# bioinf/Sibelia

Hardware: AMD Instinct MI355X
Metric: k-mers/sec in BlockFinder graph-build+simplify, 8xE.coli k=25 (higher is better)
Workload: dtype u64; 1 GPU; 8 synthetic E. coli-like strains x 4.6 Mbp (gen_strains seed 1, 1% SNP, indels, inversions), k=25 D=150 maxIterations=4, one full stage; strand_kmers_per_gpu=73598388, parallelism=1 GPU, exchange_bytes_rank0=0, bulges=334284, bif_ids=1120044, instances=7089276, rounds=106, replays=0, device_bytes=22762263122

## Files before the change

sibelia_amd/csrc/bulge_txn.h:

```cpp
#pragma once
#include <hip/hip_runtime.h>
#include <stdint.h>

#define BT_NONE 0xFFFFFFFFu
#define BT_SEP '$'
#define BT_DEAD_CHAR 0
#define BT_POS_MASK 0x1FFFFFFFu
#define BT_MAX_BREAKS 16u
#define BT_LDS_MARKS 48u
#define BT_BLOCK_SHIFT 0
#define BT_INSERT_ALIGN 1u
#define BT_RSHIFT 0u
#define BT_LAZY_MIN 64u
#define BT_MSCAN_MIN 6u
__host__ __device__ __forceinline__ uint32_t bt_insert_span(uint32_t m) { return (m + BT_INSERT_ALIGN - 1u) & ~(BT_INSERT_ALIGN - 1u); }

enum { CTR_STRIDE = 32,
       CTR_NE = 0 * CTR_STRIDE, CTR_NN = 1 * CTR_STRIDE, CTR_ERR = 2 * CTR_STRIDE, CTR_BULGES = 3 * CTR_STRIDE, CTR_VIOL = 4 * CTR_STRIDE,
       CTR_NWIN = 5 * CTR_STRIDE, CTR_LO = 6 * CTR_STRIDE, CTR_COMMITTED = 7 * CTR_STRIDE, CTR_BIG = 8 * CTR_STRIDE, CTR_PUSHED = 9 * CTR_STRIDE,
       CTR_TXN = 10 * CTR_STRIDE, CTR_DETAIL = 11 * CTR_STRIDE, CTR_COUNT = 12 * CTR_STRIDE };
enum { CTR_VDETAIL = CTR_DETAIL + 0, CTR_VDETAIL_N = 5,
       CTR_DENSE_ITER = CTR_DETAIL + 0,
       CTR_PARKED = CTR_DETAIL + 8,
       CTR_PLIST = CTR_DETAIL + 10,
// ... 351 lines not shown
	uint32_t mks;
	bool mk_overflow;
	uint32_t *wst; char *wck;
	uint32_t *wbk, *wnb;
	uint32_t *wdel;
	unsigned long long *dirty_big;
	bool lite;
	bool lazy;
	bool use_stale;
	unsigned long long stale[4];
	uint32_t epoch, *wep;
	uint32_t req[2], nreq;
	bool jscan, jready;
	uint32_t nold;
	bool mscan, mready;
	bool wfill; uint32_t fill_i;
	bool pscan, pready, pjknown; uint32_t pj;
	uint32_t ret0;
	uint32_t mscan_min;
	uint32_t mq_i, mq_di, mq_j, mq_dj, mres[2];
	uint64_t *visit; uint32_t nvisit, visit_cap;
	uint32_t *occ; uint32_t occ_cap;
	uint32_t *lb, *lf;
	AnyBulgesOut ab;
	ABuild abb;
	uint32_t gi, idI, idJ, ret;
	bool inI, need_fill;
	uint32_t c_src, c_dS, c_tgt, c_dT;
	uint32_t *act;
};
// ... 687 lines not shown
```

sibelia_amd/csrc/commit.hip:

```cpp
#include <cstring>
#include <algorithm>
#include <vector>
#include <hip/hip_runtime.h>
__device__ unsigned long long g_phase_cycles[32];
#if defined(__HIP_DEVICE_COMPILE__)
#define BT_PROF_T0(t) do { if ((t).prof) (t).prof_t = __builtin_readcyclecounter(); } while (0)
#define BT_PROF_ADD(t, i) do { if ((t).prof) { unsigned long long n_ = __builtin_readcyclecounter(); atomicAdd(&g_phase_cycles[i], n_ - (t).prof_t); (t).prof_t = n_; } } while (0)
#endif
#include "simplify_walks.h"

__device__ __forceinline__ void wave_stamp_id_write(const GraphView &g, unsigned stampv, unsigned tid, unsigned id, unsigned b)
{
	unsigned r = g.nblk + b;
	unsigned ow = g.own[b], wm = g.wmax[r], rm = g.rmax[r];
	bool bad = (stampv != BT_NONE && ow != stampv) || wm > tid || rm > tid;
	atomicMax(&g.wmax[r], tid);
	if (bad) {
		atomicMin(&g.ctr[CTR_VIOL], id);
		if (atomicCAS(&g.ctr[CTR_VDETAIL], 0u, 3u) == 0u) { g.ctr[CTR_VDETAIL + 1] = r; g.ctr[CTR_VDETAIL + 2] = (wm > rm ? wm : rm) - 1; g.ctr[CTR_VDETAIL + 3] = id; g.ctr[CTR_VDETAIL + 4] = (wm > tid ? 1u : 0u) | (rm > tid ? 2u : 0u) | (ow != stampv ? 4u : 0u); }
	}
}
__device__ __forceinline__ void wave_erase(const GraphView &g, Txn &t, unsigned strand, unsigned e, unsigned stampv, unsigned b, unsigned nd)
{
	if (b == BT_NONE) return;
// ... 1027 lines not shown
	WSYNC();
	PC_ADD(18);
	return sh.mode == 3;
	}
}


#define PARK_OFF_LAYOUT (PARK_IMG - 16u)
#define PARK_OFF_W ((unsigned)((sizeof(Txn) + 15u) & ~15u))
#define PARK_OFF_AB (PARK_OFF_W + (unsigned)((sizeof(BulgeWork) + 15u) & ~15u))
#define PARK_OFF_FAST (PARK_OFF_AB + (unsigned)((sizeof(ABShared) + 15u) & ~15u))
static_assert(sizeof(Txn) % 4 == 0 && sizeof(BulgeWork) % 4 == 0 && sizeof(ABShared) % 4 == 0, "park_move copies words");
static_assert(PARK_OFF_FAST + COMMIT_FAST_BYTES <= PARK_OFF_LAYOUT, "the LDS image of a transaction must fit PARK_IMG");
__device__ __forceinline__ unsigned lds_addr(const void *p) { return (unsigned)(uintptr_t)(const __attribute__((address_space(3))) void *)p; }
__device__ __forceinline__ void park_move(unsigned *dst, const unsigned *src, unsigned words, unsigned lane) { for (unsigned i = lane; i < words; i += 64) dst[i] = src[i]; }
__device__ __forceinline__ void park_store(const GraphView &g, Txn &t, BulgeWork &w, ABShared &absh, uint8_t *fast, unsigned fast_bytes, uint8_t *image, unsigned id, unsigned slice)
{
	const unsigned lane = threadIdx.x;
	WSYNC();
	park_move(reinterpret_cast<unsigned *>(image), reinterpret_cast<const unsigned *>(&t), sizeof(Txn) / 4, lane);
	park_move(reinterpret_cast<unsigned *>(image + PARK_OFF_W), reinterpret_cast<const unsigned *>(&w), sizeof(BulgeWork) / 4, lane);
	park_move(reinterpret_cast<unsigned *>(image + PARK_OFF_AB), reinterpret_cast<const unsigned *>(&absh), sizeof(ABShared) / 4, lane);
	park_move(reinterpret_cast<unsigned *>(image + PARK_OFF_FAST), reinterpret_cast<const unsigned *>(fast), fast_bytes / 4, lane);
	if (lane == 0) {
		unsigned *lay = reinterpret_cast<unsigned *>(image + PARK_OFF_LAYOUT);
		lay[0] = lds_addr(&t); lay[1] = lds_addr(&w); lay[2] = lds_addr(&absh); lay[3] = lds_addr(fast);
		g.park_of[id] = (slice + 1u) | (bt_round_tag(g) << 20); g.slice_busy[slice] = 1; g.need[id] = 2; atomicAdd(&g.ctr[CTR_PARKED], 1u);
#ifdef SBL_DBG_IDRET
		if (id < (1u << 20)) atomicCAS(&g_dbg_park[id], 0u, ((SS_ROUND_MAX - (g.round_bits >> 20)) << 8) | (w.ret & 255u));
#endif
	}
}
__device__ __forceinline__ bool park_load(const GraphView &g, Txn &t, BulgeWork &w, ABShared &absh, uint8_t *fast, unsigned fast_bytes, const uint8_t *image, unsigned id, unsigned wi, int prof)
{
	const unsigned lane = threadIdx.x;
	{
		const unsigned *lay = reinterpret_cast<const unsigned *>(image + PARK_OFF_LAYOUT);
		const bool same = lay[0] == lds_addr(&t) && lay[1] == lds_addr(&w) && lay[2] == lds_addr(&absh) && lay[3] == lds_addr(fast);
		if (!same) { if (lane == 0) atomicOr(&g.ctr[CTR_ERR], BT_ERR_LAYOUT); return false; }
	}
	park_move(reinterpret_cast<unsigned *>(&t), reinterpret_cast<const unsigned *>(image), sizeof(Txn) / 4, lane);
	park_move(reinterpret_cast<unsigned *>(&w), reinterpret_cast<const unsigned *>(image + PARK_OFF_W), sizeof(BulgeWork) / 4, lane);
	park_move(reinterpret_cast<unsigned *>(&absh), reinterpret_cast<const unsigned *>(image + PARK_OFF_AB), sizeof(ABShared) / 4, lane);
	park_move(reinterpret_cast<unsigned *>(fast), reinterpret_cast<const unsigned *>(image + PARK_OFF_FAST), fast_bytes / 4, lane);
	WSYNC();
	if (lane == 0) { t.g = g; t.stamp = g.round_bits | wi; t.prof = prof != 0; w.ret0 = w.ret - 1; atomicSub(&g.ctr[CTR_PARKED], 1u); }
	WSYNC();
	return true;
}
template <bool RESUME = false>
__device__ __forceinline__ void commit_body(const GraphView &g, Txn &t, BulgeWork &w, int &flag, ABShared &absh, uint8_t *fast, unsigned fast_bytes,
                                            unsigned wi, unsigned id, unsigned stampv, int solo, bool prepass, uint8_t *mine, unsigned arena_bytes, int prof,
                                            const unsigned *sepl = nullptr ,
                                            unsigned park_slice = BT_NONE )
{
	const unsigned lane = threadIdx.x, tid = id + 1;
	PH_T0();
	const bool can_park = park_slice != BT_NONE && g.park_cap != 0 && arena_bytes >= 4u * PARK_IMG;
	if (can_park) arena_bytes -= PARK_IMG;
	if (lane == 0) { g.need[id] = 0; g.touch[id] = 1; flag = 1; }
	if (RESUME) {
		if (!park_load(g, t, w, absh, fast, fast_bytes, mine + arena_bytes, id, wi, prof)) return;
		if (lane == 0) flag = 1;
		WSYNC();
	} else {
	if (prepass) {
		if (lane == 0) { t.init(g, id, wi, 1, mine, arena_bytes); t.ext_stamps = true; t.chain = stampv == BT_NONE; }
		WSYNC();
		wave_setup(g, t, w, true, lane, flag);
		if (flag) {
			wave_scan_all(g, w, lane, stampv, tid, 1, id);
			WSYNC();
		}
		int verdict = flag ? wave_verdict(g, w, *reinterpret_cast<VerdictTable *>(fast), lane) : 0;
		if (lane == 0) {
			bool has = verdict > 0;
			if (verdict < 0) { bt_end_chars(t, w); has = bt_any_bulges(t, w, true); }
			if (t.err & BT_ERR_SCRATCH) { atomicOr(&g.ctr[CTR_ERR], BT_ERR_SCRATCH); has = false; }
			flag = has ? 1 : 0;
		}
	}
	WSYNC();
	if (!flag) { if (lane == 0) { atomicAdd(&g.ctr[CTR_COMMITTED], 1u); atomicAdd(&g.ctr[CTR_TXN], 1u); } return; }
	if (lane == 0) { t.init(g, id, wi, 2, mine, arena_bytes); t.chain = stampv == BT_NONE; t.defer_push = true; t.ext_stamps = true; t.fscr = fast; t.fscr_cap = fast_bytes; w.ret = 0;
	                 t.tc_cap = 1024; t.tc_list = (uint32_t *)t.alloc(t.tc_cap * 4); if (!t.tc_list) t.tc_cap = 0; t.err = 0; t.defer_cleanup = true; t.prof = prof != 0; }
	WSYNC();
	PH_ADD(7);
	{
		const unsigned h0 = g.head[0][t.id], h1 = g.head[1][t.id];
		if (lane == 0) flag = bt_setup(t, w, false, false) && !t.err ? 1 : 0;
		WSYNC();
		PH_ADD(19);
		if (flag) {
			const unsigned m = wave_list_positions(g, h0, h1, w, lane);
			if (m != w.n && lane == 0) {
				if (t.g.any_parked && m < w.n) { w.n = m; if (m < 2) flag = 0; }
				else { t.err |= BT_ERR_SCRATCH; flag = 0; }
			}
			WSYNC();
		}
	}
	}
	PH_ADD(0);
	if (flag) {
		if (!RESUME) {
		wave_scan_all(g, w, lane, stampv, tid, 2, id);
		WSYNC();
		if (w.mk_overflow) {
			WSYNC();
			if (lane == 0) bt_marks_to_arena(t, w);
			WSYNC();
			if (!t.err) for (unsigned i = 0; i < w.n; i++) wave_scan_instance(g, w, i, lane, stampv, tid, 2, id);
			WSYNC();
		}
		PH_ADD(1);
		int any = wave_any_bulges(g, t, w, absh, lane, false, AB_COUNT_SLOTS, nullptr, prof);
		if (lane == 0) { flag = bt_rb_begin(t, w, any) && !t.err ? 1 : 0; w.lazy = solo && w.wep != nullptr; w.jscan = w.lazy || w.n > 24u; w.mscan = w.n > 24u;
			                 w.use_stale = !w.lazy && w.n <= 256u && w.wdel != nullptr; w.wfill = true; w.pscan = false; }
		WSYNC();
		PH_ADD(2);
		}
		bool decided = RESUME;
		while (flag) {
			if (!RESUME || !decided) {
			if (lane == 0) { const int r = bt_scratch_in_lds(w) ? bt_rb_run<true>(t, w) : bt_rb_run<false>(t, w); flag = t.err ? 0 : r; }
			WSYNC();
			PH_ADD(3);
			if (!flag) break;
			if (flag == 3) { wave_next_j(g, w, lane); PH_ADD(24); continue; }
			if (flag == 4) { wave_mults(g, t, w, lane); PH_ADD(25); continue; }
			if (flag == 5) { wave_fill_visit(t, w, g.D, lane); PH_ADD(26); if (t.err) break; continue; }
			if (flag == 2) {
				const unsigned nr = w.nreq;
				for (unsigned x = 0; x < nr; x++) wave_scan_instance(g, w, w.req[x], lane, stampv, tid, 2, id);
				WSYNC();
				if (lane == 0) for (unsigned x = 0; x < nr; x++) { if (w.lazy) w.wep[w.req[x]] = w.epoch; else w.stale[w.req[x] >> 6] &= ~(1ull << (w.req[x] & 63u)); }
				WSYNC();
				if (!w.lazy && w.mk_overflow) {
					if (lane == 0) bt_marks_to_arena(t, w);
					WSYNC();
					if (t.err) break;
					for (unsigned i = 0; i < w.n; i++) wave_scan_instance(g, w, i, lane, stampv, tid, 2, id);
					if (lane == 0) w.stale[0] = w.stale[1] = w.stale[2] = w.stale[3] = 0;
					WSYNC();
				}
				PH_ADD(8);
				continue;
			}
			}
			decided = false;
			if (can_park && !t.g.park_hold && !w.lazy && w.ret - w.ret0 > g.park_cap) {
				park_store(g, t, w, absh, fast, fast_bytes, mine + arena_bytes, id, park_slice);
				return;
			}
#ifdef SBL_DBG_IDRET
			if (lane == 0) {
				const unsigned o = atomicAdd(&g_dbg_nlog, 1u);
				if (o < (1u << 20)) { unsigned *r = g_dbg_log + (size_t)o * 8u; r[0] = id; r[1] = SS_ROUND_MAX - (g.round_bits >> 20); r[2] = w.ret; r[3] = (g.nslot[w.start[w.c_src] >> 1] << 1) | (w.start[w.c_src] & 1u); r[4] = (g.nslot[w.start[w.c_tgt] >> 1] << 1) | (w.start[w.c_tgt] & 1u); r[5] = w.c_dS; r[6] = w.c_dT; r[7] = RESUME ? 1u : 0u; }
			}
#endif
			if (w.lazy) {
				wave_collapse_any(g, t, w, lane, stampv, prof);
				PH_ADD(5);
				if (t.err) break;
				wave_publish_collapse(g, id, t.push_e, t.push_d, t.push_len, lane, sepl);
				if (lane == 0) w.epoch++;
				WSYNC();
				PH_ADD(6);
				continue;
			}
			unsigned long long dirty[4] = {0, 0, 0, 0};
			const bool big = w.n > 256, selective = !big || w.dirty_big != nullptr;
			if (selective) {
// ... 85 lines not shown
			unsigned long long dur = __builtin_readcyclecounter() - ph_start;
			unsigned bin = 0;
			while (bin < 15 && (dur >> (13 + bin))) bin++;
			atomicAdd(&g_txn_hist[w.ret < 3 ? w.ret : 3][bin], 1ull);
			if (atomicMax(&g_txn_max[0], dur) < dur) g_txn_max[1] = ((unsigned long long)w.n << 32) | w.ret;
			{
				const unsigned long long now = wall_clock64(), sl = (g.tslot >> 2) & 4095u;
				atomicMin(&g_round_span[3 * sl], ph_wall); atomicMax(&g_round_span[3 * sl + 1], now);
				atomicMax(&g_round_span[3 * sl + 2], ((now - ph_wall) << 32) | (ph_wall & 0xFFFFFFFFull));
				if (w.ret <= 1) atomicMax(&g_round_few[2 * sl], now - ph_wall);
				if (w.ret <= 2) atomicMax(&g_round_few[2 * sl + 1], now - ph_wall);
			}
			atomicMax(&g_round_max[(g.tslot >> 2) & 4095u], (dur << 24) | ((unsigned long long)(w.n < 255u ? w.n : 255u) << 16) | ((unsigned long long)(w.nold < 255u ? w.nold : 255u) << 8) | (w.ret < 255u ? w.ret : 255u));
		}
		atomicAdd(&g.ctr[CTR_COMMITTED], 1u); atomicAdd(&g.ctr[CTR_TXN], 1u);
		if (RESUME) { __threadfence(); g.slice_busy[park_slice] = 0; g.park_of[id] = 0x80000000u | (bt_round_tag(g) << 20); }
		if (t.err) {
			if (!t.wrote && t.err == BT_ERR_SCRATCH) { ss_mark_big(g, id); return; }
			atomicOr(&g.ctr[CTR_ERR], t.err);
		}
		atomicAdd(&g.ctr[CTR_BULGES], w.ret);
#ifdef SBL_DBG_IDRET
		if (id < (1u << 20)) { atomicAdd(&g_dbg_ret[id], w.ret); atomicCAS(&g_dbg_fin[id], 0u, ((SS_ROUND_MAX - (g.round_bits >> 20)) << 8) | (RESUME ? 128u : 0u) | (w.ret & 127u)); }
#endif
	}
}

template <bool RESUME_KERNEL>
__device__ __forceinline__ void commit_kernel(const GraphView &g, unsigned nwin, uint8_t *arena, unsigned arena_bytes, int solo, const unsigned *claims, const uint8_t *live, int prof_every)
{
	const int prof = prof_every && blockIdx.x % (unsigned)prof_every == 0u;
	__shared__ Txn t;
	__shared__ BulgeWork w;
	__shared__ int flag;
	__shared__ ABShared absh;
	__shared__ __attribute__((aligned(16))) uint8_t fast[COMMIT_FAST_BYTES];
	unsigned wi = blockIdx.x;
	const unsigned lane = threadIdx.x;
	if (!RESUME_KERNEL) round_stamp(g, 2);
	if (RESUME_KERNEL) {
		if (wi >= __builtin_amdgcn_readfirstlane((int)g.ctr[CTR_PLIST])) return;
		wi = (unsigned)__builtin_amdgcn_readfirstlane((int)g.park_list[wi]);
	}
	if (wi >= nwin) return;
	if (!solo && !live[wi]) return;
	const unsigned id = g.win[wi], stampv = g.round_bits | wi;
	if (!solo) {
		const unsigned *cb = claims + (size_t)wi * (CLAIM_CAP + 1);
		unsigned n = cb[0];
		bool owner = true;
		if (n <= CLAIM_CAP) {
			for (unsigned i = lane; i < n; i += 64) {
				unsigned b = cb[1 + i];
				if (b & 0x80000000u) { if (bt_order_blocked(g, b & 0x7FFFFFFFu)) owner = false; }
				else if (g.own[b] != stampv) owner = false;
			}
			owner = !__any(!owner);
		} else {
			if (lane == 0) owner = ss_owns_footprint(g, wi);
			owner = __shfl((int)owner, 0) != 0;
		}
		if (!owner) return;
	}
	__shared__ unsigned s_sep[64];
	const unsigned *sepl = g.sep && g.nsep <= 64 ? s_sep : nullptr;
	if (sepl) s_sep[lane] = lane < g.nsep ? g.sep[lane] : BT_NONE;
	if (RESUME_KERNEL) {
		const unsigned pk = (unsigned)__builtin_amdgcn_readfirstlane((int)g.park_of[id]);
		if (!pk || (pk >> 31) || ((pk >> 20) & 0x7FFu) == bt_round_tag(g)) return;
		const unsigned slice = (pk & 0xFFFFFu) - 1u;
		commit_body<true>(g, t, w, flag, absh, fast, (unsigned)sizeof fast, wi, id, stampv, 0, false, arena + (size_t)slice * arena_bytes, arena_bytes, prof, sepl, slice);
	} else {
		if (!solo && g.park_cap) {
			const unsigned pk = (unsigned)__builtin_amdgcn_readfirstlane((int)g.park_of[id]);
			if (pk && (!(pk >> 31) || ((pk >> 20) & 0x7FFu) == bt_round_tag(g))) return;
		}
		const bool shadow = !solo && g.park_cap && __builtin_amdgcn_readfirstlane((int)g.slice_busy[g.shadow_base + 64u + wi]) != 0;
		commit_body<false>(g, t, w, flag, absh, fast, (unsigned)sizeof fast, wi, id, stampv, solo, solo != 0, arena + (size_t)(shadow ? g.shadow_base + wi : wi) * arena_bytes, arena_bytes, prof, sepl,
		                   !solo && g.park_cap && !shadow ? wi : (unsigned)BT_NONE);
	}
}
__global__ void __launch_bounds__(64) __attribute__((amdgpu_waves_per_eu(4, 4))) k_commit(GraphView g, unsigned nwin, uint8_t *arena, unsigned arena_bytes, int solo, const unsigned *claims, const uint8_t *live, int prof_every)
{
	commit_kernel<false>(g, nwin, arena, arena_bytes, solo, claims, live, prof_every);
}

__global__ void __launch_bounds__(64) __attribute__((amdgpu_waves_per_eu(4, 4))) k_resume(GraphView g, unsigned nwin, uint8_t *arena, unsigned arena_bytes, const unsigned *claims, const uint8_t *live, int prof_every)
{
	commit_kernel<true>(g, nwin, arena, arena_bytes, 0, claims, live, prof_every);
}

__global__ void __launch_bounds__(256) k_park_sweep(unsigned *__restrict__ park_of, unsigned n)
{
	const unsigned i = blockIdx.x * blockDim.x + threadIdx.x;
	if (i < n && (park_of[i] >> 31)) park_of[i] = 0u;
}

__global__ void __launch_bounds__(64) k_chain(GraphView g, uint8_t *arena, unsigned arena_bytes, unsigned nwin, int prof)
{
	__shared__ Txn t;
	__shared__ BulgeWork w;
	__shared__ int flag;
	__shared__ ABShared absh;
	__shared__ __attribute__((aligned(16))) uint8_t fast[12288];
// ... 186 lines not shown
```

sibelia_amd/csrc/simplify.hip:

```cpp
#include <cstring>
#include <algorithm>
#include <array>
#include <chrono>

#include "sbl_ctx.h"
#include "sbl_prim.h"
#include "sbl_comm.h"
#include "kmer_kernels.h"
#include "simplify_driver.h"
#include "simplify_kernels.h"

static inline unsigned nblocks(size_t n, unsigned per) { return (unsigned)((n + per - 1) / per); }

struct SimplifyHandles {
	hipStream_t park_stream = nullptr; hipEvent_t park_ev[2] = {nullptr, nullptr};
	unsigned *h_ctr = nullptr;
	unsigned *d_hctr = nullptr;
	unsigned post_seq = 0;
	hipEvent_t ev[8] = {};
	std::vector<hipEvent_t> snap_ev;
	unsigned char *h_init = nullptr;
	~SimplifyHandles()
	{
		if (park_stream) (void)hipStreamDestroy(park_stream);
		for (auto &e : park_ev) if (e) (void)hipEventDestroy(e);
		if (h_ctr) (void)hipHostFree(h_ctr);
		if (h_init) (void)hipHostFree(h_init);
		for (auto &e : ev) if (e) (void)hipEventDestroy(e);
		for (auto &e : snap_ev) (void)hipEventDestroy(e);
	}
};
struct SimplifyState : SimplifyHandles {
	DevBuf ch, op, nx, pv, nodeof[2];
	DevBuf nslot, nnext, nidst, nclr, ndead, head[2], lsize[2];
	DevBuf ctr, need, big, touch, ck_touch, own, lock, rmax, wmax, win;
	DevBuf arena, snap_arena, big_arena, claims, live, robuf, bidx, instbuf, snap_list, snap_live, park_of, slice_busy, park_list;
	DevBuf ck_ch, ck_op, ck_nx, ck_pv, ck_bif[2], ck_nodeof[2], ck_nslot, ck_nnext, ck_ndead, ck_head[2], ck_lsize[2];
	DevBuf keys, skeys, selem, sorttmp, scantmp, perm, permin;
	DevBuf nmark, maux[2], iota, sel, tstamp;
	DevBuf lin, elin, lmpos[2], lmid[2], cnt1k, off1k;
// ... 304 lines not shown
			HIP_TRY(hipGetLastError());
		}
		HIP_TRY(hipEventRecord(st->snap_ev[2 * snap_used + 1], c->stream));
		snap_used++;
	}
	void snapshots_collect()
	{
		for (unsigned i = 0; i < snap_used; i++) {
			float ms = 0;
			HIP_TRY(hipEventSynchronize(st->snap_ev[2 * i + 1]));
			HIP_TRY(hipEventElapsedTime(&ms, st->snap_ev[2 * i], st->snap_ev[2 * i + 1]));
			snapshot_ms += ms;
		}
		snap_used = 0;
	}
	void reset_round_state(bool stamps_too)
	{
		if (stamps_too && g.park_cap) {
			HIP_TRY(hipMemsetAsync(st->park_of.p, 0, ((size_t)nid_ + 1) * 4, c->stream));
			HIP_TRY(hipMemsetAsync(st->slice_busy.p, 0, park_slices, c->stream));
			parked_known = 0; g.park_hold = 0;
		}
		HIP_TRY(hipMemsetAsync(st->own.p, 0xFF, ((size_t)nid_ + 1) * 4, c->stream));
		if (stamps_too) {
			HIP_TRY(hipMemsetAsync(st->rmax.p, 0, nres * 4, c->stream));
			HIP_TRY(hipMemsetAsync(st->wmax.p, 0, nres * 4, c->stream));
			if (g.bidx) k_idx_clear_stamps<<<(idx_nblk + 255) / 256, 256, 0, c->stream>>>(st->bidx.as<unsigned long long>(), idx_nblk);
		}
	}
	void clear_counters()
	{
		k_clear_counters<<<1, 256, 0, c->stream>>>(st->ctr.as<unsigned>());
// ... 50 lines not shown
		if (hipDeviceGetAttribute(&khz, hipDeviceAttributeWallClockRate, c->device) != hipSuccess || khz <= 0) khz = 100000;
		const double ms_per_tick = 1.0 / (double)khz;
		for (uint32_t r = 0; r < ts_round; r++) {
			const unsigned long long tp = h[4 * r], tr = h[4 * r + 1], tc = h[4 * r + 2];
			const bool probed = ts_kind[r] & 1, reserved = ts_kind[r] & 2;
			if (probed) { const unsigned long long next = reserved ? tr : tc; if (next > tp && tp) probe_ms += (double)(next - tp) * ms_per_tick; }
			if (reserved && tc > tr && tr) reserve_ms += (double)(tc - tr) * ms_per_tick;
			const unsigned long long te = h[4 * r + 3];
			if ((ts_kind[r] & 4) && te > tc && tc) commit_ms += (double)(te - tc) * ms_per_tick;
		}
	}
	void probe(uint32_t nwin, uint32_t round)
	{
		g.round_bits = (SS_ROUND_MAX - round) << 20;
		g.any_parked = parked_known != 0;
		begin_round();
		solo_round = false;
		if (g.tslot < TS_CAP * 4) ts_kind.back() |= 1;
		if (split_ro()) {
			uint32_t w0 = 0, w1 = nwin;
			share(nwin, &w0, &w1);
			const uint32_t R = c->comm->n;
			const uint32_t stride = (4u + (nwin + R - 1) / R + 1u + 3u) & ~3u;
			st->robuf.ensure((size_t)R * stride + 64);
			if (w1 > w0 && g.idx_probe) k_probe_idx<<<w1 - w0, 64, pidx_lds(), c->stream>>>(g, nwin, st->live.as<uint8_t>(), w0, pidx_vbits, pidx_inst, pidx_marks, nullptr, 0u, 0);
			if (w1 > w0) k_probe<<<w1 - w0, 64 * PROBE_WAVES, 0, c->stream>>>(g, nwin, st->arena.as<uint8_t>(), arena_bytes, st->live.as<uint8_t>(), w0, 0);
			k_pack_probe<<<std::max<uint32_t>(1u, (w1 - w0 + 255) / 256), 256, 0, c->stream>>>(st->ctr.as<unsigned>(), st->live.as<uint8_t>(), w0, w1, c->comm->rank, stride, st->robuf.as<uint8_t>());
			HIP_TRY(hipGetLastError());
			allgather_slots(st->robuf.as<char>(), R, stride);
			k_apply_probe<<<(nwin + 255) / 256, 256, 0, c->stream>>>(g, nwin, st->live.as<uint8_t>(), w0, w1, st->robuf.as<uint8_t>(), stride, R);
// ... 12 lines not shown
		if (g.tslot < TS_CAP * 4) ts_kind.back() |= 2;
		const unsigned seen_bits = rsv_waves <= 2 ? 10u : 11u, list_cap = rsv_waves <= 2 ? 256u : 1024u;
		const bool handed = g.idx_probe && !split_ro() && !solo_round;
		k_reserve<<<nwin, 64 * rsv_waves, ((1u << seen_bits) + rsv_waves * list_cap) * 4, c->stream>>>(g, nwin, st->claims.as<unsigned>(), st->live.as<uint8_t>(), seen_bits, list_cap,
		                                                                                               handed ? st->instbuf.as<unsigned>() : nullptr, istride(),
		                                                                                               g.park_cap ? st->arena.as<uint8_t>() : nullptr, arena_bytes);
		HIP_TRY(hipGetLastError());
	}
	void commit(uint32_t nwin, uint32_t round, bool solo)
	{
		g.round_bits = (SS_ROUND_MAX - round) << 20;
		const bool sampled = ((round + ev_phase) & 3u) == 0;
		if (g.tslot < TS_CAP * 4) ts_kind.back() |= 4;
		if (sampled) HIP_TRY(hipEventRecord(ev[2], c->stream));
		if (solo) {
			st->big_arena.ensure(big_arena_bytes);
			k_commit<<<1, 64, 0, c->stream>>>(g, 1, st->big_arena.as<uint8_t>(), big_arena_bytes, 1, nullptr, nullptr, prof);
		} else
		{
			const bool resume = g.park_cap && parked_known != 0;
			if (g.park_cap && (round & 1023u) == 0u) k_park_sweep<<<nblocks((size_t)nid_ + 1, 256), 256, 0, c->stream>>>(st->park_of.as<unsigned>(), nid_ + 1);
			if (resume) {
				HIP_TRY(hipEventRecord(st->park_ev[0], c->stream));
				HIP_TRY(hipStreamWaitEvent(st->park_stream, st->park_ev[0], 0));
				k_resume<<<std::min<uint32_t>(parked_known, nwin), 64, 0, st->park_stream>>>(g, nwin, st->arena.as<uint8_t>(), arena_bytes, st->claims.as<unsigned>(), st->live.as<uint8_t>(), prof);
				HIP_TRY(hipEventRecord(st->park_ev[1], st->park_stream));
			}
			k_commit<<<nwin, 64, 0, c->stream>>>(g, nwin, st->arena.as<uint8_t>(), arena_bytes, 0, st->claims.as<unsigned>(), st->live.as<uint8_t>(), prof);
			if (resume) HIP_TRY(hipStreamWaitEvent(c->stream, st->park_ev[1], 0));
		}
		if (sampled) HIP_TRY(hipEventRecord(ev[3], c->stream));
		timed_commit = sampled;
		HIP_TRY(hipGetLastError());
	}
	size_t park_slices = 0;
	uint32_t parked_known = 0;
	bool chain(uint32_t nwin, uint32_t round)
	{
		if (may_try_dense && ++chain_rounds >= 32u) {
			const double el = std::chrono::duration<double>(std::chrono::steady_clock::now() - t_stage).count();
			const double within = (double)last_lo / (double)(nid_ ? nid_ : 1u);
			const double progress = iter_count <= 1u ? 0.8 * within : 0.8 + 0.2 * ((double)(iter_count - 2u) + within) / (double)(max_iter_ > 1u ? max_iter_ - 1u : 1u);
			if (el > 1.0 && progress < 0.4) throw TryDense{};
		}
		if (g.park_cap && parked_known) { g.park_hold = 1; return false; }
		g.round_bits = (SS_ROUND_MAX - round) << 20;
		st->big_arena.ensure(big_arena_bytes);
		if (g.tslot < TS_CAP * 4) ts_kind.back() |= 4;
		k_chain<<<1, 64, 0, c->stream>>>(g, st->big_arena.as<uint8_t>(), big_arena_bytes, nwin, prof);
		timed_commit = false;
		HIP_TRY(hipGetLastError());
		return true;
	}
	SimplifyCounters counters()
	{
		read_ctr();
		if (sel_pending) sel_ready = true;
		float ms = 0;
		if (timed_commit) {
			hipError_t e = hipEventElapsedTime(&ms, ev[2], ev[3]);
			if (e == hipErrorNotReady) { HIP_TRY(hipEventSynchronize(ev[3])); e = hipEventElapsedTime(&ms, ev[2], ev[3]); }
			HIP_TRY(e);
			commit_event_ms += ms; commit_event_launches++; timed_commit = false;
		}
		SimplifyCounters r;
		memcpy(r.v, st->h_ctr, sizeof r.v);
		parked_known = r.v[CTR_PARKED];
		return r;
	}
	bool grow(uint32_t err)
	{
		if (err & ~(uint32_t)(BT_ERR_ELEM_CAP | BT_ERR_NODE_CAP)) return false;
		if (optimistic) {
			if (err & BT_ERR_ELEM_CAP) c->hint_elem_slack = std::max<size_t>(c->hint_elem_slack, 2 * ((size_t)cap_e - ne0_));
// ... 207 lines not shown
		be.ev_phase = c->stage_seq++;
		be.prof = sw.phases;
		if (be.prof) sbl_commit_prof_reset();
		if (dense) be.use_index = false;
		be.idx_nblk = be.use_index ? (uint32_t)((E + 63) / 64) : 0u;
		if (be.idx_nblk) st->bidx.ensure((size_t)be.idx_nblk * BT_IDX_WORDS * 8);
		be.bind();
		be.g.k = k; be.g.D = D;
	}

	void setup_park()
	{
		be.g.park_cap = park_cap; be.g.park_of = nullptr; be.g.slice_busy = nullptr; be.g.shadow_base = 0; be.park_slices = 0;
		be.g.park_hold = 0; be.g.any_parked = 0; be.g.park_list = nullptr;
		if (!park_cap) return;
		if (!st->park_stream) { HIP_TRY(hipStreamCreateWithFlags(&st->park_stream, hipStreamNonBlocking)); for (auto &e : st->park_ev) HIP_TRY(hipEventCreateWithFlags(&e, hipEventDisableTiming)); }
		st->park_of.ensure(((size_t)be.nid_ + 1) * 4);
		be.park_slices = (size_t)window_max + 64;
		be.g.park_of = st->park_of.as<unsigned>(); be.g.slice_busy = st->slice_busy.as<uint8_t>(); be.g.shadow_base = window_max;
		be.g.park_list = st->park_list.as<unsigned>();
	}

	bool run_dense(SimplifyReport &rep, sbl_progress_fn progress, void *user)
	{
		be.g.lazy_min = 1;
		st->big_arena.ensure(be.big_arena_bytes);
		unsigned *d_out = st->ctr.as<unsigned>() + CTR_DENSE_ITER;
		HIP_TRY(hipEventRecord(be.ev[2], s));
		k_dense_stage<<<1, 64, 0, s>>>(be.g, st->big_arena.as<uint8_t>(), be.big_arena_bytes, max_iter, d_out);
		HIP_TRY(hipEventRecord(be.ev[3], s));
		HIP_TRY(hipGetLastError());
// ... 179 lines not shown
```

sibelia_amd/csrc/simplify_kernels.h:

```cpp
#pragma once
#include "sbl_ctx.h"
#include "simplify_steps.h"

#define CLAIM_CAP 4096u
#define PROBE_WAVES 1u
#define PROBE_UNSERVED 3u
#define SEL_THREADS 256
#define RSV_WAVES_MAX 4u
struct MarkStream { const unsigned *elem[2], *id[2], *aux[2]; unsigned n[2]; };

void sbl_commit_prof_reset();
void sbl_commit_prof_report(unsigned ts_round);
void sbl_rounds_stats_report();

__global__ void __launch_bounds__(256) k_init_links(unsigned *__restrict__ nx, unsigned *__restrict__ pv, unsigned *__restrict__ nodeof0,
                                                    unsigned *__restrict__ nodeof1, uint8_t *__restrict__ ch, size_t E, size_t cap);
__global__ void __launch_bounds__(256) k_instance_keys(const unsigned *__restrict__ elem, const unsigned *__restrict__ id, unsigned n, unsigned strand,
                                                       const unsigned *__restrict__ sepidx, unsigned nchr, unsigned E, unsigned ordbits,
                                                       unsigned long long *__restrict__ keys, unsigned *__restrict__ midx);
__global__ void __launch_bounds__(256) k_build_lists(const unsigned long long *__restrict__ skeys, const unsigned *__restrict__ smidx, const unsigned *__restrict__ melem, unsigned n,
                                                     unsigned node_base, unsigned strand, unsigned ordbits, unsigned *__restrict__ nslot, unsigned *__restrict__ nnext, unsigned *__restrict__ nidst,
                                                     uint8_t *__restrict__ ndead, unsigned *__restrict__ head, unsigned *__restrict__ lsize,
                                                     unsigned *__restrict__ nodeof, unsigned *__restrict__ nmark);
__global__ void __launch_bounds__(256) k_id_position_keys(const unsigned *__restrict__ head0, const unsigned *__restrict__ head1, const unsigned *__restrict__ nslot,
// ... 14 lines not shown
__global__ void __launch_bounds__(64) k_snapshot(GraphView g, uint8_t *arena, unsigned arena_bytes, int incremental, const unsigned *__restrict__ perm, unsigned plo, unsigned phi);
__global__ void __launch_bounds__(64) k_probe_idx(GraphView g, unsigned nwin, uint8_t *live, unsigned w0, unsigned vbits, unsigned max_inst, unsigned walk_marks,
                                                  unsigned *__restrict__ instbuf, unsigned istride, int snapshot);
__global__ void __launch_bounds__(64 * PROBE_WAVES) k_probe(GraphView g, unsigned nwin, uint8_t *arena, unsigned arena_bytes, uint8_t *live, unsigned w0, int snapshot);
__global__ void __launch_bounds__(256) k_pack_need(const unsigned *__restrict__ perm, const uint8_t *__restrict__ need, unsigned lo, unsigned hi, uint8_t *__restrict__ buf);
__global__ void __launch_bounds__(256) k_unpack_need(const unsigned *__restrict__ perm, const uint8_t *__restrict__ buf, unsigned n, unsigned mylo, unsigned myhi, uint8_t *__restrict__ need);
__global__ void __launch_bounds__(256) k_apply_probe(GraphView g, unsigned nwin, uint8_t *__restrict__ live, unsigned w0, unsigned w1, const uint8_t *__restrict__ robuf, unsigned stride, unsigned nranks);
__global__ void __launch_bounds__(SEL_THREADS) k_select_count(GraphView g, unsigned *__restrict__ sel, unsigned lo, unsigned limit, unsigned chunk0, unsigned chunk,
                                                              const uint8_t *__restrict__ live, unsigned probed);
__global__ void __launch_bounds__(SEL_THREADS) k_select_write(GraphView g, unsigned *__restrict__ sel, unsigned *__restrict__ win, unsigned lo, unsigned limit, unsigned W,
                                                              unsigned chunk0, unsigned chunk, unsigned nchunks, volatile unsigned *post, unsigned post_seq);
__global__ void __launch_bounds__(256) k_pack_probe(const unsigned *__restrict__ ctr, const uint8_t *__restrict__ live, unsigned w0, unsigned w1, unsigned rank, unsigned stride, uint8_t *__restrict__ robuf);
__global__ void __launch_bounds__(64 * RSV_WAVES_MAX) k_reserve(GraphView g, unsigned nwin, unsigned *claims, const uint8_t *live, unsigned seen_bits, unsigned list_cap,
                                                                 const unsigned *__restrict__ instbuf, unsigned istride, const uint8_t *arena, unsigned arena_bytes);
__global__ void __launch_bounds__(64) __attribute__((amdgpu_waves_per_eu(4, 4))) k_commit(GraphView g, unsigned nwin, uint8_t *arena, unsigned arena_bytes, int solo, const unsigned *claims, const uint8_t *live, int prof);
__global__ void __launch_bounds__(64) __attribute__((amdgpu_waves_per_eu(4, 4))) k_resume(GraphView g, unsigned nwin, uint8_t *arena, unsigned arena_bytes, const unsigned *claims, const uint8_t *live, int prof);
__global__ void __launch_bounds__(256) k_park_sweep(unsigned *__restrict__ park_of, unsigned n);
__global__ void __launch_bounds__(64) k_chain(GraphView g, uint8_t *arena, unsigned arena_bytes, unsigned nwin, int prof);
__global__ void __launch_bounds__(64) k_dense_stage(GraphView g, uint8_t *arena, unsigned arena_bytes, unsigned max_iter, unsigned *out);
__global__ void __launch_bounds__(256) k_count_touched(const uint8_t *__restrict__ touch, unsigned nid, unsigned *__restrict__ out);
__global__ void __launch_bounds__(256) k_touched_list(const uint8_t *__restrict__ touch, unsigned nid, unsigned *__restrict__ list, unsigned *__restrict__ count);
__global__ void __launch_bounds__(256) k_seg_flags(const uint8_t *__restrict__ ch, const unsigned *__restrict__ nx, unsigned ne, unsigned *__restrict__ flag);
__global__ void __launch_bounds__(256) k_seg_tails(const uint8_t *__restrict__ ch, const unsigned *__restrict__ nx, unsigned ne,
                                                   const unsigned *__restrict__ flag, const unsigned *__restrict__ segidx ,
                                                   unsigned *__restrict__ seg_head, unsigned *__restrict__ seg_len, unsigned *__restrict__ seg_succ_elem);
__global__ void __launch_bounds__(256) k_seg_finish(unsigned nseg, const unsigned *__restrict__ seg_head, unsigned *__restrict__ seg_len,
                                                    const unsigned *__restrict__ seg_succ_elem, const unsigned *__restrict__ flag,
                                                    const unsigned *__restrict__ segidx, unsigned *__restrict__ succ, unsigned long long *__restrict__ dist);
__global__ void __launch_bounds__(256) k_seg_jump(unsigned nseg, const unsigned *__restrict__ succ_in, const unsigned long long *__restrict__ dist_in,
                                                  unsigned *__restrict__ succ_out, unsigned long long *__restrict__ dist_out);
__global__ void __launch_bounds__(256) k_scatter_linear(const uint8_t *__restrict__ ch, const unsigned *__restrict__ op, unsigned ne,
// ... 19 lines not shown
```

Before: 1.310 billion strand-k-mers/s.

## Merge resume kernel into commit kernel and drop separate park stream

The separate k_resume kernel, which ran on its own stream with event handoffs, is folded into k_commit. The first blocks of the combined grid resume parked transactions and the rest run fresh windows. Resume/park state moves from a template parameter into runtime fields on BulgeWork, and the GraphView is read through the kernarg pointer. Park sweep is moved into the round-reset and round-start paths. The aim is to remove the extra stream, event record/wait and a launch per round, at the cost of runtime branching and register pressure in a single unified kernel.

Result: faster. 1.373 billion strand-k-mers/s, median of 6 (+4.8%).

```diff
diff --git a/sibelia_amd/csrc/bulge_txn.h b/sibelia_amd/csrc/bulge_txn.h
--- a/sibelia_amd/csrc/bulge_txn.h
+++ b/sibelia_amd/csrc/bulge_txn.h
@@ -389,6 +389,8 @@
 	bool jscan, jready;
 	uint32_t nold;
 	bool mscan, mready;
+	uint8_t resumed;
+	bool can_park;
 	bool wfill; uint32_t fill_i;
 	bool pscan, pready, pjknown; uint32_t pj;
 	uint32_t ret0;
diff --git a/sibelia_amd/csrc/commit.hip b/sibelia_amd/csrc/commit.hip
--- a/sibelia_amd/csrc/commit.hip
+++ b/sibelia_amd/csrc/commit.hip
@@ -1065,10 +1065,11 @@
 static_assert(PARK_OFF_FAST + COMMIT_FAST_BYTES <= PARK_OFF_LAYOUT, "the LDS image of a transaction must fit PARK_IMG");
 __device__ __forceinline__ unsigned lds_addr(const void *p) { return (unsigned)(uintptr_t)(const __attribute__((address_space(3))) void *)p; }
 __device__ __forceinline__ void park_move(unsigned *dst, const unsigned *src, unsigned words, unsigned lane) { for (unsigned i = lane; i < words; i += 64) dst[i] = src[i]; }
-__device__ __forceinline__ void park_store(const GraphView &g, Txn &t, BulgeWork &w, ABShared &absh, uint8_t *fast, unsigned fast_bytes, uint8_t *image, unsigned id, unsigned slice)
+__device__ __forceinline__ void park_store(const GraphView &g, Txn &t, BulgeWork &w, ABShared &absh, uint8_t *fast, unsigned fast_bytes, unsigned id)
 {
 	const unsigned lane = threadIdx.x;
 	WSYNC();
+	uint8_t *image = t.scr + t.scr_cap;
 	park_move(reinterpret_cast<unsigned *>(image), reinterpret_cast<const unsigned *>(&t), sizeof(Txn) / 4, lane);
 	park_move(reinterpret_cast<unsigned *>(image + PARK_OFF_W), reinterpret_cast<const unsigned *>(&w), sizeof(BulgeWork) / 4, lane);
 	park_move(reinterpret_cast<unsigned *>(image + PARK_OFF_AB), reinterpret_cast<const unsigned *>(&absh), sizeof(ABShared) / 4, lane);
@@ -1076,6 +1077,7 @@
 	if (lane == 0) {
 		unsigned *lay = reinterpret_cast<unsigned *>(image + PARK_OFF_LAYOUT);
 		lay[0] = lds_addr(&t); lay[1] = lds_addr(&w); lay[2] = lds_addr(&absh); lay[3] = lds_addr(fast);
+		const unsigned slice = w.resumed ? (g.park_of[id] & 0xFFFFFu) - 1u : t.stamp & 0xFFFFFu;
 		g.park_of[id] = (slice + 1u) | (bt_round_tag(g) << 20); g.slice_busy[slice] = 1; g.need[id] = 2; atomicAdd(&g.ctr[CTR_PARKED], 1u);
 #ifdef SBL_DBG_IDRET
 		if (id < (1u << 20)) atomicCAS(&g_dbg_park[id], 0u, ((SS_ROUND_MAX - (g.round_bits >> 20)) << 8) | (w.ret & 255u));
@@ -1095,22 +1097,22 @@
 	park_move(reinterpret_cast<unsigned *>(&absh), reinterpret_cast<const unsigned *>(image + PARK_OFF_AB), sizeof(ABShared) / 4, lane);
 	park_move(reinterpret_cast<unsigned *>(fast), reinterpret_cast<const unsigned *>(image + PARK_OFF_FAST), fast_bytes / 4, lane);
 	WSYNC();
-	if (lane == 0) { t.g = g; t.stamp = g.round_bits | wi; t.prof = prof != 0; w.ret0 = w.ret - 1; atomicSub(&g.ctr[CTR_PARKED], 1u); }
+	if (lane == 0) { t.g = g; t.stamp = g.round_bits | wi; t.prof = prof != 0; w.ret0 = w.ret - 1; w.resumed = 3; atomicSub(&g.ctr[CTR_PARKED], 1u); }
 	WSYNC();
 	return true;
 }
-template <bool RESUME = false>
 __device__ __forceinline__ void commit_body(const GraphView &g, Txn &t, BulgeWork &w, int &flag, ABShared &absh, uint8_t *fast, unsigned fast_bytes,
                                             unsigned wi, unsigned id, unsigned stampv, int solo, bool prepass, uint8_t *mine, unsigned arena_bytes, int prof,
                                             const unsigned *sepl = nullptr ,
-                                            unsigned park_slice = BT_NONE )
+                                            bool own_slice = false ,
+                                            bool resume = false )
 {
 	const unsigned lane = threadIdx.x, tid = id + 1;
 	PH_T0();
-	const bool can_park = park_slice != BT_NONE && g.park_cap != 0 && arena_bytes >= 4u * PARK_IMG;
+	const bool can_park = (own_slice || resume) && g.park_cap != 0 && arena_bytes >= 4u * PARK_IMG;
 	if (can_park) arena_bytes -= PARK_IMG;
 	if (lane == 0) { g.need[id] = 0; g.touch[id] = 1; flag = 1; }
-	if (RESUME) {
+	if (resume) {
 		if (!park_load(g, t, w, absh, fast, fast_bytes, mine + arena_bytes, id, wi, prof)) return;
 		if (lane == 0) flag = 1;
 		WSYNC();
@@ -1133,7 +1135,7 @@
 	}
 	WSYNC();
 	if (!flag) { if (lane == 0) { atomicAdd(&g.ctr[CTR_COMMITTED], 1u); atomicAdd(&g.ctr[CTR_TXN], 1u); } return; }
-	if (lane == 0) { t.init(g, id, wi, 2, mine, arena_bytes); t.chain = stampv == BT_NONE; t.defer_push = true; t.ext_stamps = true; t.fscr = fast; t.fscr_cap = fast_bytes; w.ret = 0;
+	if (lane == 0) { t.init(g, id, wi, 2, mine, arena_bytes); t.chain = stampv == BT_NONE; t.defer_push = true; t.ext_stamps = true; t.fscr = fast; t.fscr_cap = fast_bytes; w.ret = 0; w.resumed = 0; w.can_park = can_park;
 	                 t.tc_cap = 1024; t.tc_list = (uint32_t *)t.alloc(t.tc_cap * 4); if (!t.tc_list) t.tc_cap = 0; t.err = 0; t.defer_cleanup = true; t.prof = prof != 0; }
 	WSYNC();
 	PH_ADD(7);
@@ -1154,7 +1156,7 @@
 	}
 	PH_ADD(0);
 	if (flag) {
-		if (!RESUME) {
+		if (!w.resumed) {
 		wave_scan_all(g, w, lane, stampv, tid, 2, id);
 		WSYNC();
 		if (w.mk_overflow) {
@@ -1171,10 +1173,11 @@
 		WSYNC();
 		PH_ADD(2);
 		}
-		bool decided = RESUME;
 		while (flag) {
-			if (!RESUME || !decided) {
-			if (lane == 0) { const int r = bt_scratch_in_lds(w) ? bt_rb_run<true>(t, w) : bt_rb_run<false>(t, w); flag = t.err ? 0 : r; }
+			if (lane == 0) {
+				if (w.resumed & 2u) { w.resumed = 1; flag = 1; }
+				else { const int r = bt_scratch_in_lds(w) ? bt_rb_run<true>(t, w) : bt_rb_run<false>(t, w); flag = t.err ? 0 : r; }
+			}
 			WSYNC();
 			PH_ADD(3);
 			if (!flag) break;
@@ -1198,16 +1201,14 @@
 				PH_ADD(8);
 				continue;
 			}
-			}
-			decided = false;
-			if (can_park && !t.g.park_hold && !w.lazy && w.ret - w.ret0 > g.park_cap) {
-				park_store(g, t, w, absh, fast, fast_bytes, mine + arena_bytes, id, park_slice);
+			if (w.can_park && !t.g.park_hold && !w.lazy && w.ret - w.ret0 > g.park_cap) {
+				park_store(g, t, w, absh, fast, fast_bytes, id);
 				return;
 			}
 #ifdef SBL_DBG_IDRET
 			if (lane == 0) {
 				const unsigned o = atomicAdd(&g_dbg_nlog, 1u);
-				if (o < (1u << 20)) { unsigned *r = g_dbg_log + (size_t)o * 8u; r[0] = id; r[1] = SS_ROUND_MAX - (g.round_bits >> 20); r[2] = w.ret; r[3] = (g.nslot[w.start[w.c_src] >> 1] << 1) | (w.start[w.c_src] & 1u); r[4] = (g.nslot[w.start[w.c_tgt] >> 1] << 1) | (w.start[w.c_tgt] & 1u); r[5] = w.c_dS; r[6] = w.c_dT; r[7] = RESUME ? 1u : 0u; }
+				if (o < (1u << 20)) { unsigned *r = g_dbg_log + (size_t)o * 8u; r[0] = id; r[1] = SS_ROUND_MAX - (g.round_bits >> 20); r[2] = w.ret; r[3] = (g.nslot[w.start[w.c_src] >> 1] << 1) | (w.start[w.c_src] & 1u); r[4] = (g.nslot[w.start[w.c_tgt] >> 1] << 1) | (w.start[w.c_tgt] & 1u); r[5] = w.c_dS; r[6] = w.c_dT; r[7] = w.resumed ? 1u : 0u; }
 			}
 #endif
 			if (w.lazy) {
@@ -1323,33 +1324,36 @@
 			atomicMax(&g_round_max[(g.tslot >> 2) & 4095u], (dur << 24) | ((unsigned long long)(w.n < 255u ? w.n : 255u) << 16) | ((unsigned long long)(w.nold < 255u ? w.nold : 255u) << 8) | (w.ret < 255u ? w.ret : 255u));
 		}
 		atomicAdd(&g.ctr[CTR_COMMITTED], 1u); atomicAdd(&g.ctr[CTR_TXN], 1u);
-		if (RESUME) { __threadfence(); g.slice_busy[park_slice] = 0; g.park_of[id] = 0x80000000u | (bt_round_tag(g) << 20); }
+		if (w.resumed) { __threadfence(); g.slice_busy[(g.park_of[id] & 0xFFFFFu) - 1u] = 0; g.park_of[id] = 0x80000000u | (bt_round_tag(g) << 20); }
 		if (t.err) {
 			if (!t.wrote && t.err == BT_ERR_SCRATCH) { ss_mark_big(g, id); return; }
 			atomicOr(&g.ctr[CTR_ERR], t.err);
 		}
 		atomicAdd(&g.ctr[CTR_BULGES], w.ret);
 #ifdef SBL_DBG_IDRET
-		if (id < (1u << 20)) { atomicAdd(&g_dbg_ret[id], w.ret); atomicCAS(&g_dbg_fin[id], 0u, ((SS_ROUND_MAX - (g.round_bits >> 20)) << 8) | (RESUME ? 128u : 0u) | (w.ret & 127u)); }
+		if (id < (1u << 20)) { atomicAdd(&g_dbg_ret[id], w.ret); atomicCAS(&g_dbg_fin[id], 0u, ((SS_ROUND_MAX - (g.round_bits >> 20)) << 8) | (w.resumed ? 128u : 0u) | (w.ret & 127u)); }
 #endif
 	}
 }
 
-template <bool RESUME_KERNEL>
-__device__ __forceinline__ void commit_kernel(const GraphView &g, unsigned nwin, uint8_t *arena, unsigned arena_bytes, int solo, const unsigned *claims, const uint8_t *live, int prof_every)
-{
+__global__ void __launch_bounds__(64) __attribute__((amdgpu_waves_per_eu(4, 4))) k_commit(GraphView g_arg, unsigned nwin, uint8_t *arena, unsigned arena_bytes, int solo, const unsigned *claims, const uint8_t *live, int prof_every)
+{
+	(void)g_arg;
+	const GraphView &g = *(const GraphView *)(const __attribute__((address_space(4))) GraphView *)__builtin_amdgcn_kernarg_segment_ptr();
 	const int prof = prof_every && blockIdx.x % (unsigned)prof_every == 0u;
 	__shared__ Txn t;
 	__shared__ BulgeWork w;
 	__shared__ int flag;
 	__shared__ ABShared absh;
 	__shared__ __attribute__((aligned(16))) uint8_t fast[COMMIT_FAST_BYTES];
-	unsigned wi = blockIdx.x;
+	const unsigned nres = solo ? 0u : gridDim.x - nwin;
+	const bool resume = blockIdx.x < nres;
+	unsigned wi = blockIdx.x - nres;
 	const unsigned lane = threadIdx.x;
-	if (!RESUME_KERNEL) round_stamp(g, 2);
-	if (RESUME_KERNEL) {
-		if (wi >= __builtin_amdgcn_readfirstlane((int)g.ctr[CTR_PLIST])) return;
-		wi = (unsigned)__builtin_amdgcn_readfirstlane((int)g.park_list[wi]);
+	round_stamp(g, 2);
+	if (resume) {
+		if (blockIdx.x >= (unsigned)__builtin_amdgcn_readfirstlane((int)g.ctr[CTR_PLIST])) return;
+		wi = (unsigned)__builtin_amdgcn_readfirstlane((int)g.park_list[blockIdx.x]);
 	}
 	if (wi >= nwin) return;
 	if (!solo && !live[wi]) return;
@@ -1374,29 +1378,18 @@
 	__shared__ unsigned s_sep[64];
 	const unsigned *sepl = g.sep && g.nsep <= 64 ? s_sep : nullptr;
 	if (sepl) s_sep[lane] = lane < g.nsep ? g.sep[lane] : BT_NONE;
-	if (RESUME_KERNEL) {
+	unsigned slice = wi; bool own_slice = false;
+	if (!solo && g.park_cap) {
 		const unsigned pk = (unsigned)__builtin_amdgcn_readfirstlane((int)g.park_of[id]);
-		if (!pk || (pk >> 31) || ((pk >> 20) & 0x7FFu) == bt_round_tag(g)) return;
-		const unsigned slice = (pk & 0xFFFFFu) - 1u;
-		commit_body<true>(g, t, w, flag, absh, fast, (unsigned)sizeof fast, wi, id, stampv, 0, false, arena + (size_t)slice * arena_bytes, arena_bytes, prof, sepl, slice);
-	} else {
-		if (!solo && g.park_cap) {
-			const unsigned pk = (unsigned)__builtin_amdgcn_readfirstlane((int)g.park_of[id]);
+		if (resume) {
+			if (!pk || (pk >> 31) || ((pk >> 20) & 0x7FFu) == bt_round_tag(g)) return;
+			slice = (pk & 0xFFFFFu) - 1u;
+		} else {
 			if (pk && (!(pk >> 31) || ((pk >> 20) & 0x7FFu) == bt_round_tag(g))) return;
-		}
-		const bool shadow = !solo && g.park_cap && __builtin_amdgcn_readfirstlane((int)g.slice_busy[g.shadow_base + 64u + wi]) != 0;
-		commit_body<false>(g, t, w, flag, absh, fast, (unsigned)sizeof fast, wi, id, stampv, solo, solo != 0, arena + (size_t)(shadow ? g.shadow_base + wi : wi) * arena_bytes, arena_bytes, prof, sepl,
-		                   !solo && g.park_cap && !shadow ? wi : (unsigned)BT_NONE);
-	}
-}
-__global__ void __launch_bounds__(64) __attribute__((amdgpu_waves_per_eu(4, 4))) k_commit(GraphView g, unsigned nwin, uint8_t *arena, unsigned arena_bytes, int solo, const unsigned *claims, const uint8_t *live, int prof_every)
-{
-	commit_kernel<false>(g, nwin, arena, arena_bytes, solo, claims, live, prof_every);
-}
-
-__global__ void __launch_bounds__(64) __attribute__((amdgpu_waves_per_eu(4, 4))) k_resume(GraphView g, unsigned nwin, uint8_t *arena, unsigned arena_bytes, const unsigned *claims, const uint8_t *live, int prof_every)
-{
-	commit_kernel<true>(g, nwin, arena, arena_bytes, 0, claims, live, prof_every);
+			if (__builtin_amdgcn_readfirstlane((int)g.slice_busy[g.shadow_base + 64u + wi]) != 0) slice = g.shadow_base + wi; else own_slice = true;
+		}
+	}
+	commit_body(g, t, w, flag, absh, fast, (unsigned)sizeof fast, wi, id, stampv, solo, solo != 0, arena + (size_t)slice * arena_bytes, arena_bytes, prof, sepl, own_slice, resume);
 }
 
 __global__ void __launch_bounds__(256) k_park_sweep(unsigned *__restrict__ park_of, unsigned n)
diff --git a/sibelia_amd/csrc/simplify.hip b/sibelia_amd/csrc/simplify.hip
--- a/sibelia_amd/csrc/simplify.hip
+++ b/sibelia_amd/csrc/simplify.hip
@@ -13,7 +13,6 @@
 static inline unsigned nblocks(size_t n, unsigned per) { return (unsigned)((n + per - 1) / per); }
 
 struct SimplifyHandles {
-	hipStream_t park_stream = nullptr; hipEvent_t park_ev[2] = {nullptr, nullptr};
 	unsigned *h_ctr = nullptr;
 	unsigned *d_hctr = nullptr;
 	unsigned post_seq = 0;
@@ -22,8 +21,6 @@
 	unsigned char *h_init = nullptr;
 	~SimplifyHandles()
 	{
-		if (park_stream) (void)hipStreamDestroy(park_stream);
-		for (auto &e : park_ev) if (e) (void)hipEventDestroy(e);
 		if (h_ctr) (void)hipHostFree(h_ctr);
 		if (h_init) (void)hipHostFree(h_init);
 		for (auto &e : ev) if (e) (void)hipEventDestroy(e);
@@ -358,8 +355,10 @@
 		}
 		snap_used = 0;
 	}
+	void park_sweep() { if (g.park_cap) k_park_sweep<<<nblocks((size_t)nid_ + 1, 256), 256, 0, c->stream>>>(st->park_of.as<unsigned>(), nid_ + 1); }
 	void reset_round_state(bool stamps_too)
 	{
+		if (!stamps_too) park_sweep();
 		if (stamps_too && g.park_cap) {
 			HIP_TRY(hipMemsetAsync(st->park_of.p, 0, ((size_t)nid_ + 1) * 4, c->stream));
 			HIP_TRY(hipMemsetAsync(st->slice_busy.p, 0, park_slices, c->stream));
@@ -440,6 +439,7 @@
 	{
 		g.round_bits = (SS_ROUND_MAX - round) << 20;
 		g.any_parked = parked_known != 0;
+		if ((round & 1023u) == 0u) park_sweep();
 		begin_round();
 		solo_round = false;
 		if (g.tslot < TS_CAP * 4) ts_kind.back() |= 1;
@@ -482,20 +482,12 @@
 		if (g.tslot < TS_CAP * 4) ts_kind.back() |= 4;
 		if (sampled) HIP_TRY(hipEventRecord(ev[2], c->stream));
 		if (solo) {
+			if ((round & 1023u) == 0u) park_sweep();
 			st->big_arena.ensure(big_arena_bytes);
 			k_commit<<<1, 64, 0, c->stream>>>(g, 1, st->big_arena.as<uint8_t>(), big_arena_bytes, 1, nullptr, nullptr, prof);
-		} else
-		{
-			const bool resume = g.park_cap && parked_known != 0;
-			if (g.park_cap && (round & 1023u) == 0u) k_park_sweep<<<nblocks((size_t)nid_ + 1, 256), 256, 0, c->stream>>>(st->park_of.as<unsigned>(), nid_ + 1);
-			if (resume) {
-				HIP_TRY(hipEventRecord(st->park_ev[0], c->stream));
-				HIP_TRY(hipStreamWaitEvent(st->park_stream, st->park_ev[0], 0));
-				k_resume<<<std::min<uint32_t>(parked_known, nwin), 64, 0, st->park_stream>>>(g, nwin, st->arena.as<uint8_t>(), arena_bytes, st->claims.as<unsigned>(), st->live.as<uint8_t>(), prof);
-				HIP_TRY(hipEventRecord(st->park_ev[1], st->park_stream));
-			}
-			k_commit<<<nwin, 64, 0, c->stream>>>(g, nwin, st->arena.as<uint8_t>(), arena_bytes, 0, st->claims.as<unsigned>(), st->live.as<uint8_t>(), prof);
-			if (resume) HIP_TRY(hipStreamWaitEvent(c->stream, st->park_ev[1], 0));
+		} else {
+			const uint32_t nresume = g.park_cap ? std::min<uint32_t>(parked_known, nwin) : 0u;
+			k_commit<<<nresume + nwin, 64, 0, c->stream>>>(g, nwin, st->arena.as<uint8_t>(), arena_bytes, 0, st->claims.as<unsigned>(), st->live.as<uint8_t>(), prof);
 		}
 		if (sampled) HIP_TRY(hipEventRecord(ev[3], c->stream));
 		timed_commit = sampled;
@@ -524,8 +516,8 @@
 	{
 		read_ctr();
 		if (sel_pending) sel_ready = true;
-		float ms = 0;
 		if (timed_commit) {
+			float ms = 0;
 			hipError_t e = hipEventElapsedTime(&ms, ev[2], ev[3]);
 			if (e == hipErrorNotReady) { HIP_TRY(hipEventSynchronize(ev[3])); e = hipEventElapsedTime(&ms, ev[2], ev[3]); }
 			HIP_TRY(e);
@@ -763,7 +755,6 @@
 		be.g.park_cap = park_cap; be.g.park_of = nullptr; be.g.slice_busy = nullptr; be.g.shadow_base = 0; be.park_slices = 0;
 		be.g.park_hold = 0; be.g.any_parked = 0; be.g.park_list = nullptr;
 		if (!park_cap) return;
-		if (!st->park_stream) { HIP_TRY(hipStreamCreateWithFlags(&st->park_stream, hipStreamNonBlocking)); for (auto &e : st->park_ev) HIP_TRY(hipEventCreateWithFlags(&e, hipEventDisableTiming)); }
 		st->park_of.ensure(((size_t)be.nid_ + 1) * 4);
 		be.park_slices = (size_t)window_max + 64;
 		be.g.park_of = st->park_of.as<unsigned>(); be.g.slice_busy = st->slice_busy.as<uint8_t>(); be.g.shadow_base = window_max;
diff --git a/sibelia_amd/csrc/simplify_kernels.h b/sibelia_amd/csrc/simplify_kernels.h
--- a/sibelia_amd/csrc/simplify_kernels.h
+++ b/sibelia_amd/csrc/simplify_kernels.h
@@ -52,7 +52,6 @@
 __global__ void __launch_bounds__(64 * RSV_WAVES_MAX) k_reserve(GraphView g, unsigned nwin, unsigned *claims, const uint8_t *live, unsigned seen_bits, unsigned list_cap,
                                                                  const unsigned *__restrict__ instbuf, unsigned istride, const uint8_t *arena, unsigned arena_bytes);
 __global__ void __launch_bounds__(64) __attribute__((amdgpu_waves_per_eu(4, 4))) k_commit(GraphView g, unsigned nwin, uint8_t *arena, unsigned arena_bytes, int solo, const unsigned *claims, const uint8_t *live, int prof);
-__global__ void __launch_bounds__(64) __attribute__((amdgpu_waves_per_eu(4, 4))) k_resume(GraphView g, unsigned nwin, uint8_t *arena, unsigned arena_bytes, const unsigned *claims, const uint8_t *live, int prof);
 __global__ void __launch_bounds__(256) k_park_sweep(unsigned *__restrict__ park_of, unsigned n);
 __global__ void __launch_bounds__(64) k_chain(GraphView g, uint8_t *arena, unsigned arena_bytes, unsigned nwin, int prof);
 __global__ void __launch_bounds__(64) k_dense_stage(GraphView g, uint8_t *arena, unsigned arena_bytes, unsigned max_iter, unsigned *out);
```
